# microsoft/MaskFlownet

Hardware: NVIDIA H100
Metric: image-pairs/sec (MaskFlownet-S forward, 1024x448) (higher is better)
Workload: dtype f32

## Files before the change

maskflownet_b200/csrc/api.cu:

```cuda
#include <atomic>
#include <cstdarg>
#include <cstdio>
#include <cstring>

#include "common.cuh"

namespace mfn {

static thread_local char g_err[512] = "";
static thread_local const char* g_kernel = "";
static std::atomic<unsigned long long> g_launches{0};

int fail(int code, const char* fmt, ...) {
  va_list ap;
  va_start(ap, fmt);
  vsnprintf(g_err, sizeof(g_err), fmt, ap);
  va_end(ap);
  return code;
}

void note_kernel(const char* name) { g_kernel = name; }

Tuning& tuning() {
  static Tuning t;
  return t;
}

int check_launch(const char* kernel_name) {
  const cudaError_t e = cudaGetLastError();
  if (e != cudaSuccess) return fail((int)e, "%s: launch failed: %s", kernel_name, cudaGetErrorString(e));
  g_kernel = kernel_name;
  g_launches.fetch_add(1, std::memory_order_relaxed);
  g_err[0] = '\0';
  return MFN_OK;
}

}

extern "C" int mfn_version(void) { return MFN_VERSION; }
extern "C" const char* mfn_last_error(void) { return mfn::g_err; }
extern "C" const char* mfn_last_kernel(void) { return mfn::g_kernel; }
extern "C" unsigned long long mfn_launch_count(void) { return mfn::g_launches.load(std::memory_order_relaxed); }

extern "C" int mfn_set_tuning(const char* key, int value) {
  if (!key) return mfn::fail(MFN_ERR_INVALID_ARG, "mfn_set_tuning: null key");
  if (!strcmp(key, "corr_grid_cap")) mfn::tuning().corr_grid_cap = value;
  else if (!strcmp(key, "corr_disable_ring")) mfn::tuning().corr_disable_ring = value;
  else if (!strcmp(key, "warp_lin")) mfn::tuning().warp_lin = value;
  else if (!strcmp(key, "corr_rb")) mfn::tuning().corr_rb = value;
  else if (!strcmp(key, "warp_lin_fch")) mfn::tuning().warp_lin_fch = value;
  else if (!strcmp(key, "conv_as")) mfn::tuning().conv_as = value;
  else if (!strcmp(key, "conv_splitk")) mfn::tuning().conv_splitk = value;
  else if (!strcmp(key, "conv_narrow")) mfn::tuning().conv_narrow = value;
  else if (!strcmp(key, "conv_tma_in")) mfn::tuning().conv_tma_in = value;
  else if (!strcmp(key, "corr_rb_twb")) mfn::tuning().corr_rb_twb = value;
  else if (!strcmp(key, "corr_rb_rows")) mfn::tuning().corr_rb_rows = value;
  else if (!strcmp(key, "corr_tma")) mfn::tuning().corr_tma = value;
  else if (!strcmp(key, "corr_ts_lo")) mfn::tuning().corr_ts_lo = value;
  else if (!strcmp(key, "corr_ts_hi")) mfn::tuning().corr_ts_hi = value;
  else if (!strcmp(key, "corr_dbg")) mfn::tuning().corr_dbg = value;
  else if (!strcmp(key, "conv_dbg")) mfn::tuning().conv_dbg = value;
  else if (!strcmp(key, "corr_ring_th")) mfn::tuning().corr_ring_th = value;
  else if (!strcmp(key, "conv_wgmma")) mfn::tuning().conv_wgmma = value;
  else if (!strcmp(key, "conv_grid_cap")) mfn::tuning().conv_grid_cap = value;
  else if (!strcmp(key, "conv_wgmma_min_w")) mfn::tuning().conv_wgmma_min_w = value;
  else return mfn::fail(MFN_ERR_INVALID_ARG, "mfn_set_tuning: unknown key '%s'", key);
  return MFN_OK;
}
```

maskflownet_b200/csrc/common.cuh:

```cuda
#pragma once
#include <cuda_runtime.h>
#include <stdint.h>

#include "../../include/maskflow_b200.h"
#include "device_caps.h"
#include "sampling.cuh"

namespace mfn {

int fail(int code, const char* fmt, ...);
int check_launch(const char* kernel_name);
void note_kernel(const char* name);

struct Tuning {
  int corr_grid_cap = 0;
  int corr_disable_ring = 0;
  int conv_wgmma = 1;
  int conv_grid_cap = 0;
  int conv_wgmma_min_w = 1;
  int corr_ring_th = 8;
  int corr_rb = 1;
  int warp_lin_fch = 0;
  int conv_as = 0;
  int conv_splitk = 1;
  int conv_narrow = 1;
  int conv_tma_in = 1;
  int corr_rb_twb = 0;
  int corr_rb_rows = 0;
  int corr_tma = 1;
  int warp_lin = 1;
  int corr_ts_lo = 0, corr_ts_hi = 0;
  int corr_dbg = 0;
  int conv_dbg = 0;
};
Tuning& tuning();

static inline cudaStream_t as_stream(void* s) { return reinterpret_cast<cudaStream_t>(s); }

#define MFN_REQUIRE(cond, code, ...)                   \
  do {                                                 \
    if (!(cond)) return ::mfn::fail(code, __VA_ARGS__); \
  } while (0)

static inline bool aligned(const void* p, size_t a) { return (reinterpret_cast<uintptr_t>(p) % a) == 0; }

static inline unsigned grid_for(long long total, int threads) {
  long long b = (total + threads - 1) / threads;
  const long long cap = (long long)kNumSMs * 16;
  return (unsigned)(b < cap ? (b > 0 ? b : 1) : cap);
}


struct SmemOptIn {
  int bytes[64] = {};
};
template <typename K>
static inline cudaError_t ensure_dyn_smem(K kernel, int bytes, SmemOptIn& st) {
  int dev = 0;
  if (cudaGetDevice(&dev) != cudaSuccess) dev = -1;
  if (dev >= 0 && dev < 64 && st.bytes[dev] >= bytes) return cudaSuccess;
  const cudaError_t e = cudaFuncSetAttribute(kernel, cudaFuncAttributeMaxDynamicSharedMemorySize, bytes);
  if (e == cudaSuccess && dev >= 0 && dev < 64) st.bytes[dev] = bytes;
  return e;
}

long long warp_lin_workspace_bytes(int N, int F, int H, int W);
int launch_warp_lin(const float* x, const float* flow_c, const float* mask_c, const float* weight, const void* packed_weight,
                    const float* bias, const float* tradeoff, void* workspace, float* out, float* fup, float* mup, int N,
                    int C, int H, int W, int F, int up, float fs, float ls, float slope, int border_mode, cudaStream_t st);

int launch_corr_rb(int md, const float* d1, const float* d2, float* out, int N, int C, int H, int W, long long obs,
                   float slope, cudaStream_t st);

int launch_corr_tma(int md, const float* d1, const float* d2, float* out, int N, int C, int H, int W, long long obs,
                    float slope, cudaStream_t st);

int det_launch_abs_max(const float* v, long long n, unsigned* bound, cudaStream_t st);
int det_launch_pixel_abs_sum_max(const float* g, int N, int F, long long HW, unsigned* bound, cudaStream_t st);
int det_launch_fixed_to_float(const unsigned long long* acc, float* out, long long n, const unsigned* bound, int nb,
// ... 75 lines not shown
```

maskflownet_b200/csrc/conv3x3_wgmma.cu:

```cuda
#include <cstring>
#include <type_traits>

#include "mma_tiles.cuh"
#include "split_act.cuh"

namespace mfn {
namespace um {
constexpr int MT_WIDE = 128, MT_NARROW = 64;
inline int tile_width(int OW, int stride) {
  return tuning().conv_narrow && (OW <= MT_NARROW || (stride == 2 && tuning().conv_tma_in)) ? MT_NARROW : MT_WIDE;
}
constexpr int R = 2;
constexpr int NTHREADS = 384;
constexpr int NCONS = 8;
constexpr int NPROD = 3;
constexpr int MAX_AS = 4, MAX_WS = 24;
constexpr int MAX_RS = 4;
constexpr int BATCH = 6;
constexpr int BAR_BYTES = 1024;

__host__ __device__ inline int n_slots(int stride, int dil) { return stride == 2 ? 2 * R + 1 : (dil >= R ? 3 * R : R + 2 * dil); }
__host__ __device__ inline int row_pitch(int mt, int stride, int dil) { return stride == 2 ? 2 * mt + 1 : mt + 2 * dil; }
__host__ __device__ inline int slot_of(int r, int ky, int stride, int dil) {
  return stride == 2 ? 2 * r + ky : (dil >= R ? ky * R + r : r + ky * dil);
// ... 56 lines not shown
  static_assert(S >= 32, "accumulator too small");
  asm volatile(
      "{\n\t.reg .pred p;\n\tsetp.ne.b32 p, %34, 0;\n\t"
      "wgmma.mma_async.sync.aligned.m64n64k16.f32.bf16.bf16 {%0, %1, %2, %3, %4, %5, %6, %7, %8, %9, %10, %11, %12, %13, %14, %15, %16, %17, %18, %19, %20, %21, %22, %23, %24, %25, %26, %27, %28, %29, %30, %31}, %32, %33, p, 1, 1, 0, 0;\n\t}"
      : "+f"(d[0]), "+f"(d[1]), "+f"(d[2]), "+f"(d[3]), "+f"(d[4]), "+f"(d[5]), "+f"(d[6]), "+f"(d[7]), "+f"(d[8]), "+f"(d[9]), "+f"(d[10]), "+f"(d[11]), "+f"(d[12]), "+f"(d[13]), "+f"(d[14]), "+f"(d[15]), "+f"(d[16]), "+f"(d[17]), "+f"(d[18]), "+f"(d[19]), "+f"(d[20]), "+f"(d[21]), "+f"(d[22]), "+f"(d[23]), "+f"(d[24]), "+f"(d[25]), "+f"(d[26]), "+f"(d[27]), "+f"(d[28]), "+f"(d[29]), "+f"(d[30]), "+f"(d[31])
      : "l"(a), "l"(b), "r"(scale_d));
}
template <int S>
__device__ __forceinline__ void wgmma_n80(float (&d)[S], uint64_t a, uint64_t b, uint32_t scale_d) {
  static_assert(S >= 40, "accumulator too small");
  asm volatile(
      "{\n\t.reg .pred p;\n\tsetp.ne.b32 p, %42, 0;\n\t"
      "wgmma.mma_async.sync.aligned.m64n80k16.f32.bf16.bf16 {%0, %1, %2, %3, %4, %5, %6, %7, %8, %9, %10, %11, %12, %13, %14, %15, %16, %17, %18, %19, %20, %21, %22, %23, %24, %25, %26, %27, %28, %29, %30, %31, %32, %33, %34, %35, %36, %37, %38, %39}, %40, %41, p, 1, 1, 0, 0;\n\t}"
      : "+f"(d[0]), "+f"(d[1]), "+f"(d[2]), "+f"(d[3]), "+f"(d[4]), "+f"(d[5]), "+f"(d[6]), "+f"(d[7]), "+f"(d[8]), "+f"(d[9]), "+f"(d[10]), "+f"(d[11]), "+f"(d[12]), "+f"(d[13]), "+f"(d[14]), "+f"(d[15]), "+f"(d[16]), "+f"(d[17]), "+f"(d[18]), "+f"(d[19]), "+f"(d[20]), "+f"(d[21]), "+f"(d[22]), "+f"(d[23]), "+f"(d[24]), "+f"(d[25]), "+f"(d[26]), "+f"(d[27]), "+f"(d[28]), "+f"(d[29]), "+f"(d[30]), "+f"(d[31]), "+f"(d[32]), "+f"(d[33]), "+f"(d[34]), "+f"(d[35]), "+f"(d[36]), "+f"(d[37]), "+f"(d[38]), "+f"(d[39])
      : "l"(a), "l"(b), "r"(scale_d));
}
template <int S>
__device__ __forceinline__ void wgmma_n96(float (&d)[S], uint64_t a, uint64_t b, uint32_t scale_d) {
  static_assert(S >= 48, "accumulator too small");
  asm volatile(
      "{\n\t.reg .pred p;\n\tsetp.ne.b32 p, %50, 0;\n\t"
      "wgmma.mma_async.sync.aligned.m64n96k16.f32.bf16.bf16 {%0, %1, %2, %3, %4, %5, %6, %7, %8, %9, %10, %11, %12, %13, %14, %15, %16, %17, %18, %19, %20, %21, %22, %23, %24, %25, %26, %27, %28, %29, %30, %31, %32, %33, %34, %35, %36, %37, %38, %39, %40, %41, %42, %43, %44, %45, %46, %47}, %48, %49, p, 1, 1, 0, 0;\n\t}"
      : "+f"(d[0]), "+f"(d[1]), "+f"(d[2]), "+f"(d[3]), "+f"(d[4]), "+f"(d[5]), "+f"(d[6]), "+f"(d[7]), "+f"(d[8]), "+f"(d[9]), "+f"(d[10]), "+f"(d[11]), "+f"(d[12]), "+f"(d[13]), "+f"(d[14]), "+f"(d[15]), "+f"(d[16]), "+f"(d[17]), "+f"(d[18]), "+f"(d[19]), "+f"(d[20]), "+f"(d[21]), "+f"(d[22]), "+f"(d[23]), "+f"(d[24]), "+f"(d[25]), "+f"(d[26]), "+f"(d[27]), "+f"(d[28]), "+f"(d[29]), "+f"(d[30]), "+f"(d[31]), "+f"(d[32]), "+f"(d[33]), "+f"(d[34]), "+f"(d[35]), "+f"(d[36]), "+f"(d[37]), "+f"(d[38]), "+f"(d[39]), "+f"(d[40]), "+f"(d[41]), "+f"(d[42]), "+f"(d[43]), "+f"(d[44]), "+f"(d[45]), "+f"(d[46]), "+f"(d[47])
      : "l"(a), "l"(b), "r"(scale_d));
}
template <int S>
__device__ __forceinline__ void wgmma_n112(float (&d)[S], uint64_t a, uint64_t b, uint32_t scale_d) {
  static_assert(S >= 56, "accumulator too small");
  asm volatile(
      "{\n\t.reg .pred p;\n\tsetp.ne.b32 p, %58, 0;\n\t"
      "wgmma.mma_async.sync.aligned.m64n112k16.f32.bf16.bf16 {%0, %1, %2, %3, %4, %5, %6, %7, %8, %9, %10, %11, %12, %13, %14, %15, %16, %17, %18, %19, %20, %21, %22, %23, %24, %25, %26, %27, %28, %29, %30, %31, %32, %33, %34, %35, %36, %37, %38, %39, %40, %41, %42, %43, %44, %45, %46, %47, %48, %49, %50, %51, %52, %53, %54, %55}, %56, %57, p, 1, 1, 0, 0;\n\t}"
      : "+f"(d[0]), "+f"(d[1]), "+f"(d[2]), "+f"(d[3]), "+f"(d[4]), "+f"(d[5]), "+f"(d[6]), "+f"(d[7]), "+f"(d[8]), "+f"(d[9]), "+f"(d[10]), "+f"(d[11]), "+f"(d[12]), "+f"(d[13]), "+f"(d[14]), "+f"(d[15]), "+f"(d[16]), "+f"(d[17]), "+f"(d[18]), "+f"(d[19]), "+f"(d[20]), "+f"(d[21]), "+f"(d[22]), "+f"(d[23]), "+f"(d[24]), "+f"(d[25]), "+f"(d[26]), "+f"(d[27]), "+f"(d[28]), "+f"(d[29]), "+f"(d[30]), "+f"(d[31]), "+f"(d[32]), "+f"(d[33]), "+f"(d[34]), "+f"(d[35]), "+f"(d[36]), "+f"(d[37]), "+f"(d[38]), "+f"(d[39]), "+f"(d[40]), "+f"(d[41]), "+f"(d[42]), "+f"(d[43]), "+f"(d[44]), "+f"(d[45]), "+f"(d[46]), "+f"(d[47]), "+f"(d[48]), "+f"(d[49]), "+f"(d[50]), "+f"(d[51]), "+f"(d[52]), "+f"(d[53]), "+f"(d[54]), "+f"(d[55])
      : "l"(a), "l"(b), "r"(scale_d));
}
template <int S>
__device__ __forceinline__ void wgmma_n128(float (&d)[S], uint64_t a, uint64_t b, uint32_t scale_d) {
  static_assert(S >= 64, "accumulator too small");
  asm volatile(
      "{\n\t.reg .pred p;\n\tsetp.ne.b32 p, %66, 0;\n\t"
      "wgmma.mma_async.sync.aligned.m64n128k16.f32.bf16.bf16 {%0, %1, %2, %3, %4, %5, %6, %7, %8, %9, %10, %11, %12, %13, %14, %15, %16, %17, %18, %19, %20, %21, %22, %23, %24, %25, %26, %27, %28, %29, %30, %31, %32, %33, %34, %35, %36, %37, %38, %39, %40, %41, %42, %43, %44, %45, %46, %47, %48, %49, %50, %51, %52, %53, %54, %55, %56, %57, %58, %59, %60, %61, %62, %63}, %64, %65, p, 1, 1, 0, 0;\n\t}"
      : "+f"(d[0]), "+f"(d[1]), "+f"(d[2]), "+f"(d[3]), "+f"(d[4]), "+f"(d[5]), "+f"(d[6]), "+f"(d[7]), "+f"(d[8]), "+f"(d[9]), "+f"(d[10]), "+f"(d[11]), "+f"(d[12]), "+f"(d[13]), "+f"(d[14]), "+f"(d[15]), "+f"(d[16]), "+f"(d[17]), "+f"(d[18]), "+f"(d[19]), "+f"(d[20]), "+f"(d[21]), "+f"(d[22]), "+f"(d[23]), "+f"(d[24]), "+f"(d[25]), "+f"(d[26]), "+f"(d[27]), "+f"(d[28]), "+f"(d[29]), "+f"(d[30]), "+f"(d[31]), "+f"(d[32]), "+f"(d[33]), "+f"(d[34]), "+f"(d[35]), "+f"(d[36]), "+f"(d[37]), "+f"(d[38]), "+f"(d[39]), "+f"(d[40]), "+f"(d[41]), "+f"(d[42]), "+f"(d[43]), "+f"(d[44]), "+f"(d[45]), "+f"(d[46]), "+f"(d[47]), "+f"(d[48]), "+f"(d[49]), "+f"(d[50]), "+f"(d[51]), "+f"(d[52]), "+f"(d[53]), "+f"(d[54]), "+f"(d[55]), "+f"(d[56]), "+f"(d[57]), "+f"(d[58]), "+f"(d[59]), "+f"(d[60]), "+f"(d[61]), "+f"(d[62]), "+f"(d[63])
      : "l"(a), "l"(b), "r"(scale_d));
}
template <int N, int S>
__device__ __forceinline__ void wgmma_bf16(float (&d)[S], uint64_t a, uint64_t b, uint32_t scale_d) {
  if constexpr (N == 16) wgmma_n16(d, a, b, scale_d);
  else if constexpr (N == 32) wgmma_n32(d, a, b, scale_d);
  else if constexpr (N == 48) wgmma_n48(d, a, b, scale_d);
  else if constexpr (N == 64) wgmma_n64(d, a, b, scale_d);
  else if constexpr (N == 80) wgmma_n80(d, a, b, scale_d);
  else if constexpr (N == 96) wgmma_n96(d, a, b, scale_d);
  else if constexpr (N == 112) wgmma_n112(d, a, b, scale_d);
  else wgmma_n128(d, a, b, scale_d);
}

struct SplitK {
  int k, from, n_lo, y_lo, rh;
  long long part_stride;
  float* ws;
  uint32_t magic_tp, magic_tx;
  int as_wide;
  int ns;
  int stg;
};
__device__ __forceinline__ void decode_tile(int tile, int tilesX, int tilesY, const SplitK& sk, int& tx, int& ty, int& n) {
  if (sk.magic_tp) {
    n = (int)__umulhi((uint32_t)tile, sk.magic_tp);
    const int rem = tile - n * tilesX * tilesY;
    ty = sk.magic_tx ? (int)__umulhi((uint32_t)rem, sk.magic_tx) : rem;
    tx = rem - ty * tilesX;
  } else {
    tx = tile % tilesX;
    ty = (tile / tilesX) % tilesY;
    n = tile / (tilesX * tilesY);
  }
}
struct SplitDev {
  int in, in_g0, in_Cg;
  unsigned char* out;
  int out_Cg, out_c0;
};
struct Work {
  int tile, part, cb, ce, nh;
};
__device__ __forceinline__ Work decode_work(int w, const SplitK& sk, int nChunks) {
  Work r;
  r.nh = 0;
  if (sk.ns == 2) {
    r.nh = w & 1;
    w >>= 1;
  }
  if (sk.k <= 1 || w < sk.from) {
    r.tile = w; r.part = -1; r.cb = 0; r.ce = nChunks;
  } else {
    const int u = w - sk.from, t = u / sk.k;
    r.tile = sk.from + t;
    r.part = u - t * sk.k;
    r.cb = r.part * nChunks / sk.k;
    r.ce = (r.part + 1) * nChunks / sk.k;
  }
  return r;
}

struct SmemMap {
  int a_lo, a_stage, w_tile, w_stage, w_off, bar_off, stg_off, total, AS, WS, raw_off, raw_stage, RS;
};
// ... 12 lines not shown
    const int raw_off = (2 * m.a_stage + 127) / 128 * 128;
    m.RS = rs_max;
    while (m.RS > 2 && budget - raw_off - m.RS * raw < 3 * m.w_stage) --m.RS;
    budget -= m.RS * raw + (raw_off - 2 * m.a_stage);
  }
  if (raw)
    m.AS = 2;
  else if (taps_per_stage(CoutP) > 1)
    m.AS = (4 * m.a_stage + 4 * m.w_stage <= budget) ? 4 : ((3 * m.a_stage + 3 * m.w_stage <= budget) ? 3 : 2);
  else
    m.AS = (as_wide >= 3 && 3 * m.a_stage + 8 * m.w_stage <= budget) ? 3 : 2;
  int ws = (budget - m.AS * m.a_stage) / m.w_stage;
  m.WS = ws > MAX_WS ? MAX_WS : ws;
  m.raw_off = raw ? (m.AS * m.a_stage + 127) / 128 * 128 : m.AS * m.a_stage;
  m.raw_stage = raw;
  m.w_off = m.raw_off + m.RS * raw;
  m.bar_off = m.w_off + m.WS * m.w_stage;
  m.stg_off = m.bar_off + BAR_BYTES;
  m.total = m.stg_off + stg;
  return m;
}
}

__global__ void conv3x3_pack_wgmma_kernel(const float* __restrict__ w, unsigned char* __restrict__ packed, int Cin, int Cout,
                                          int CoutP, int nChunks16) {
  const long long total = (long long)nChunks16 * 9 * CoutP * 8;
  for (long long i = (long long)blockIdx.x * blockDim.x + threadIdx.x; i < total; i += (long long)gridDim.x * blockDim.x) {
    const int j = (int)(i & 7);
    const int f = (int)((i >> 3) % CoutP);
    const int tap = (int)((i / (8LL * CoutP)) % 9);
    const int c = (int)(i / (8LL * CoutP * 9));
    const int ch = 16 * c + 2 * j;
    float a = 0.f, b = 0.f;
    if (f < Cout) {
      if (ch < Cin) a = w[((size_t)f * Cin + ch) * 9 + tap];
      if (ch + 1 < Cin) b = w[((size_t)f * Cin + ch + 1) * 9 + tap];
    }
    uint32_t hi, lo;
    split_pair(a, b, hi, lo);
    const int wt = 64 * CoutP;
    unsigned char* tile = packed + ((size_t)c * 9 + tap) * wt;
    if (um::fold_hi_lo(CoutP)) {
      const int off = (j >> 2) * (2 * CoutP * 16) + f * 16 + (j & 3) * 4;
      *reinterpret_cast<uint32_t*>(tile + off) = hi;
      *reinterpret_cast<uint32_t*>(tile + CoutP * 16 + off) = lo;
    } else {
      const int off = (j >> 2) * (CoutP * 16) + f * 16 + (j & 3) * 4;
      *reinterpret_cast<uint32_t*>(tile + off) = hi;
      *reinterpret_cast<uint32_t*>(tile + wt / 2 + off) = lo;
    }
  }
}

template <int NW, bool FOLD, int TPS, int TERMS, int MT>
__global__ void __launch_bounds__(um::NTHREADS, 1)
    conv3x3_wgmma_kernel(const float* __restrict__ x, long long x_bs, const unsigned char* __restrict__ wpack,
                         const float* __restrict__ bias_arg, float* __restrict__ out_base, long long out_bs, int Cin, int H, int W,
                         int OH, int OW, int Cout, int CoutP, int nChunks, float slope_arg, int tilesX, int tilesY, int numWork,
                         int stride, int dil, int out_mode_arg, int ext, um::SplitK sk, um::SplitDev xs,
                         const __grid_constant__ CUtensorMap tmx, int dbg) {
  using namespace um;
  static_assert(TERMS == 1 || TERMS == 3, "one or three products per multiply-add");
  static_assert(MT == MT_WIDE || MT == MT_NARROW, "128- or 64-pixel tile rows");
  constexpr bool FOLD_ACC = FOLD && TERMS == 3;
  constexpr int P = TERMS == 1 ? 1 : 2;
  constexpr int NCOL = FOLD_ACC ? NW / 2 : NW;
  constexpr int MB = MT / 64;
  const int out_mode_k = out_mode_arg & 0xff, lin_prefix_k = out_mode_arg >> 8;
  extern __shared__ __align__(128) unsigned char smem[];
  const int nslots = n_slots(stride, dil), PW = row_pitch(MT, stride, dil), E = nslots * PW;
  const SmemMap sm = smem_map(E, CoutP, sk.as_wide, sk.stg, TERMS, xs.in == 2 ? raw_stage_bytes(nslots, MT, stride) : 0,
                              raw_ring_max(stride));
  const int AS = sm.AS, WS = sm.WS, RS = sm.RS;
  const uint32_t s_base = smem_u32(smem);
  const uint32_t bar0 = s_base + sm.bar_off;
  const uint32_t a_full = bar0, a_empty = bar0 + 8 * MAX_AS, w_full = bar0 + 16 * MAX_AS, w_empty = w_full + 8 * MAX_WS;
  const uint32_t r_full = w_empty + 8 * MAX_WS, r_empty = r_full + 8 * MAX_RS;

  const int tid = threadIdx.x, lane = tid & 31;
  const int warp = __shfl_sync(0xffffffffu, tid >> 5, 0);
  const size_t plane = (size_t)H * W;

  if (tid == 0) {
    for (int i = 0; i < AS; ++i) {
      mbar_init(a_full + 8 * i, xs.in == 1 ? 1 : NPROD);
      mbar_init(a_empty + 8 * i, NCONS);
    }
    for (int i = 0; i < RS; ++i) {
      mbar_init(r_full + 8 * i, 1);
      mbar_init(r_empty + 8 * i, NPROD);
    }
    for (int i = 0; i < WS; ++i) {
      mbar_init(w_full + 8 * i, 1);
      mbar_init(w_empty + 8 * i, NCONS);
    }
    asm volatile("fence.mbarrier_init.release.cluster;" ::: "memory");
  }
  __syncthreads();

  if (warp < 8) {
    const int r = warp >> 2, wq = warp & 3;
    const uint32_t a_lbo = (uint32_t)E * 16u, b_lbo = (uint32_t)(FOLD_ACC ? 2 * CoutP : CoutP) * 16u;
    uint32_t a_off[9];
#pragma unroll
    for (int tap = 0; tap < 9; ++tap)
      a_off[tap] = (uint32_t)(slot_of(r, tap / 3, stride, dil) * PW + tap_xoff(MT, tap % 3, stride, dil));
    const uint64_t dh_a = desc_hi(a_lbo, 128u), dh_b = desc_hi(b_lbo, 128u);
    uint32_t as = 0, aph = 0, ws = 0, wph = 0;
    const uint32_t a_lo16 = (uint32_t)sm.a_lo >> 4, a_stage16 = (uint32_t)sm.a_stage >> 4, s_base16 = s_base >> 4;
    const uint32_t w_base16 = (s_base + (uint32_t)sm.w_off) >> 4, w_tile16 = (uint32_t)sm.w_tile >> 4, w_half16 = w_tile16 >> 1;
    const uint32_t w_stage16 = (uint32_t)sm.w_stage >> 4;
    int rel_w = -1, rel_a = -1;
    auto release = [&]() {
      if (lane == 0) {
        if (rel_w >= 0) mbar_arrive(w_empty + 8 * rel_w);
        if (rel_a >= 0) mbar_arrive(a_empty + 8 * rel_a);
      }
      rel_w = rel_a = -1;
    };
    float acc[MB][NW / 2];
    for (int work = blockIdx.x; work < numWork; work += gridDim.x) {
      const Work wk = decode_work(work, sk, nChunks);
      const int cb = wk.cb, ce = wk.ce;
      const uint32_t b_nh16 = (uint32_t)(wk.nh * NCOL);
#pragma unroll
      for (int mh = 0; mh < MB; ++mh) fence_acc(acc[mh]);
      if (dbg & 8) {
        for (int c = cb; c < ce; ++c) {
          mbar_wait(a_full + 8 * as, aph);
          for (int tap = 0; tap < 9; ++tap) {
            if (tap % TPS == 0) mbar_wait(w_full + 8 * ws, wph);
            release();
            if (tap % TPS == TPS - 1) {
              rel_w = (int)ws;
              if (++ws == (uint32_t)WS) { ws = 0; wph ^= 1; }
            }
            if (tap == 8) rel_a = (int)as;
          }
          if (++as == (uint32_t)AS) { as = 0; aph ^= 1; }
        }
      }
      for (int c = (dbg & 8) ? ce : cb; c < ce; ++c) {
        mbar_wait(a_full + 8 * as, aph);
        const uint32_t a_st16 = s_base16 + as * a_stage16;
#pragma unroll
        for (int tap = 0; tap < 9; ++tap) {
          if (tap % TPS == 0) mbar_wait(w_full + 8 * ws, wph);
          const uint32_t w16 = w_base16 + ws * w_stage16 + (uint32_t)(tap % TPS) * w_tile16 + b_nh16;
          const uint64_t b_hi = dh_b | (uint64_t)w16, b_lo = dh_b | (uint64_t)(w16 + w_half16);
          const uint32_t sc = (tap == 0 && c == cb) ? 0u : 1u;
          wgmma_fence();
#pragma unroll
          for (int mh = 0; mh < MB; ++mh) {
// ... 190 lines not shown
                bulk_g2s(dst + (uint32_t)(t * sm.w_tile + run), src + t * gt + 2 * run, (uint32_t)run, w_full + 8 * ws);
              } else {
                bulk_g2s(dst + (uint32_t)(t * sm.w_tile), src + t * gt, (uint32_t)sm.w_tile, w_full + 8 * ws);
              }
            }
            if (++ws == (uint32_t)WS) { ws = 0; wph ^= 1; wrapped = true; }
          }
        }
      }
    }
  } else {
    if (xs.in == 1) {
      if (warp == 9 && lane == 0) {
        uint32_t as = 0, aph = 0;
        bool wrapped = false;
        for (int work = blockIdx.x; work < numWork; work += gridDim.x) {
          const Work wk = decode_work(work, sk, nChunks);
          int tx, ty, n;
          decode_tile(wk.tile, tilesX, tilesY, sk, tx, ty, n);
          const int x0 = tx * MT - dil, y0 = ty * R;
          const int gb = n * P * xs.in_Cg + xs.in_g0;
          for (int c = wk.cb; c < wk.ce; ++c) {
            if (wrapped) mbar_wait(a_empty + 8 * as, aph ^ 1);
            const uint32_t bar = a_full + 8 * as, dst = s_base + as * (uint32_t)sm.a_stage;
            if (dbg & 16) {
              mbar_arrive(bar);
            } else {
              mbar_arrive_expect_tx(bar, (uint32_t)sm.a_stage);
              const int g = gb + 2 * c;
              if (dil < R) {
                tma_load_4d(dst, &tmx, 0, x0, y0 - dil, g, bar);
                if constexpr (P == 2) tma_load_4d(dst + (uint32_t)sm.a_lo, &tmx, 0, x0, y0 - dil, g + xs.in_Cg, bar);
              } else if constexpr (P == 1) {
#pragma unroll 1
                for (int k = 0; k < 6; ++k) {
                  const int ky = k >> 1, kc = k & 1;
                  tma_load_4d(dst + (uint32_t)((kc * E + ky * R * PW) * 16), &tmx, 0, x0, y0 + (ky - 1) * dil, g + kc, bar);
                }
              } else {
#pragma unroll 1
                for (int k = 0; k < 12; ++k) {
                  const int ky = k >> 2, kc = (k >> 1) & 1, pl = k & 1;
                  tma_load_4d(dst + (uint32_t)(pl * sm.a_lo + (kc * E + ky * R * PW) * 16), &tmx, 0, x0, y0 + (ky - 1) * dil,
                              g + kc + pl * xs.in_Cg, bar);
                }
              }
            }
            if (++as == (uint32_t)AS) { as = 0; aph ^= 1; wrapped = true; }
          }
        }
      }
      return;
    }
    if (dbg & 16) {
      uint32_t as = 0, aph = 0;
      bool wrapped = false;
      for (int work = blockIdx.x; work < numWork; work += gridDim.x) {
        const Work wk = decode_work(work, sk, nChunks);
        for (int c = wk.cb; c < wk.ce; ++c) {
          if (wrapped) mbar_wait(a_empty + 8 * as, aph ^ 1);
          __syncwarp();
          if (lane == 0) mbar_arrive(a_full + 8 * as);
          if (++as == (uint32_t)AS) { as = 0; aph ^= 1; wrapped = true; }
        }
      }
      return;
    }
    const int pw = warp - 9;
    const int G = (E + 31) / 32;
    const bool one_plane = Cin <= 8;
    const int nItems = one_plane ? G : 2 * G;
    const int nb = (nItems + NPROD * BATCH - 1) / (NPROD * BATCH);
    const uint32_t pw_magic = 0xFFFFFFFFu / (uint32_t)PW + 1u;
    if (one_plane) {
      for (int st = 0; st < AS; ++st)
        for (int e = pw * 32 + lane; e < E; e += NPROD * 32) {
          unsigned char* d = smem + st * sm.a_stage + (E + e) * 16;
          *reinterpret_cast<uint4*>(d) = make_uint4(0u, 0u, 0u, 0u);
          if constexpr (P == 2) *reinterpret_cast<uint4*>(d + sm.a_lo) = make_uint4(0u, 0u, 0u, 0u);
        }
    }
    if (xs.in == 2) {
      const bool s2 = stride == 2;
      const int RP = raw_pitch(MT, stride), CP = nslots * RP;
      const int RPC = s2 && !one_plane ? 2 : 1;
      const uint32_t raw_bytes = (uint32_t)sm.raw_stage, raw_base = s_base + (uint32_t)sm.raw_off;
      const bool issuer = warp == 9 && lane == 0;
      int i_work = blockIdx.x, i_c = 0, i_h = 0, i_ce = 0, i_x = 0, i_y = 0, i_n = 0;
      auto i_tile = [&]() {
        if (i_work >= numWork) return;
        const Work wk = decode_work(i_work, sk, nChunks);
        int tx, ty;
        decode_tile(wk.tile, tilesX, tilesY, sk, tx, ty, i_n);
        i_c = wk.cb;
        i_ce = wk.ce;
        i_x = s2 ? 2 * tx * MT - 4 : tx * MT - 4;
        i_y = s2 ? 2 * ty * R - 1 : ty * R - 1;
      };
      auto issue = [&](uint32_t slot) {
        if (i_work >= numWork) return;
        const uint32_t bar = r_full + 8 * slot;
        if (dbg & 2) {
          mbar_arrive(bar);
        } else {
          mbar_arrive_expect_tx(bar, raw_bytes);
          tma_load_4d(raw_base + slot * raw_bytes, &tmx, i_x, i_y, 16 * i_c + 8 * i_h, i_n, bar);
// ... 324 lines not shown
  const int as_wide = tuning().conv_as == 2 ? 2 : 3;
  const bool staged = (out_mode & 0xff) == 0 && ext == 0 &&
                      (xs.out != nullptr ? (out_mode >> 8) == 0 : OW % 4 == 0 && out_bs % 4 == 0 && aligned(out, 16)) &&
                      smem_map(E, CoutP, as_wide, STG_BYTES, terms).WS >= 2;
  int raw = 0;
  const bool raw_geometry = stride == 1 ? dil == 1 && MT == MT_WIDE : MT == MT_NARROW && OW > MT_NARROW;
  if (sio.in == nullptr && tuning().conv_tma_in && raw_geometry && ext == 0 && W % 4 == 0 && x_bs % 4 == 0 &&
      aligned(x, 16)) {
    raw = raw_stage_bytes(n_slots(stride, 1), MT, stride);
    if (smem_map(E, CoutP, as_wide, staged ? STG_BYTES : 0, terms, raw, raw_ring_max(stride)).WS < 3) raw = 0;
  }
  if (raw) {
    EncodeTiledFn fn = encode_tiled_fn();
    if (fn == nullptr) return fail(MFN_ERR_UNSUPPORTED, "cuTensorMapEncodeTiled is not available from this driver");
    const cuuint64_t dim[4] = {(cuuint64_t)W, (cuuint64_t)H, (cuuint64_t)Cin, (cuuint64_t)N};
    const cuuint64_t strides[3] = {(cuuint64_t)W * 4, (cuuint64_t)W * H * 4, (cuuint64_t)x_bs * 4};
    const cuuint32_t box[4] = {(cuuint32_t)raw_pitch(MT, stride), (cuuint32_t)n_slots(stride, 1),
                               (cuuint32_t)raw_channels(stride), 1};
    const cuuint32_t es[4] = {1, 1, 1, 1};
    const CUresult r = fn(&tmx, CU_TENSOR_MAP_DATA_TYPE_FLOAT32, 4, const_cast<float*>(x), dim, strides, box, es,
                          CU_TENSOR_MAP_INTERLEAVE_NONE, CU_TENSOR_MAP_SWIZZLE_NONE, CU_TENSOR_MAP_L2_PROMOTION_L2_256B,
                          CU_TENSOR_MAP_FLOAT_OOB_FILL_NONE);
    if (r != CUDA_SUCCESS) return fail(MFN_ERR_UNSUPPORTED, "cuTensorMapEncodeTiled failed (CUresult %d)", (int)r);
    xs.in = 2;
  }
  const SmemMap sm = smem_map(E, CoutP, as_wide, staged ? STG_BYTES : 0, terms, raw, raw_ring_max(stride));
  if (sm.WS < 2 || E * 16 > 0x3FFF * 16) return -1;
  if ((long long)H * W >= (1LL << 27)) return -1;
  const int tilesX = (OW + MT - 1) / MT, tilesY = (OH + R - 1) / R;
  const int ns = CoutP > 128 ? 2 : 1;
  SplitK sk = {1, 0, 0, 0, 0, 0, nullptr, 0u, 0u, 3, ns};
  if (ws != nullptr && ext == 0) {
    sk = plan_split(N, Cin, H, W, Cout, stride, dil, tuning().conv_grid_cap);
    if (sk.k > 1 && ws_bytes < sk.k * sk.part_stride * 4) sk.k = 1;
    sk.ws = ws;
  }
  const long long tiles = (long long)N * tilesX * tilesY;
  if (tiles * ns >= (1LL << 30)) return -1;
  sk.as_wide = as_wide;
  sk.stg = staged ? STG_BYTES : 0;
  if (sk.k <= 1) sk.from = (int)tiles;
  {
    const unsigned long long tp = (unsigned long long)tilesX * tilesY;
    if ((unsigned long long)tiles * tp < (1ull << 32) && tp * tilesX < (1ull << 32)) {
      sk.magic_tp = (uint32_t)(((1ull << 32) + tp - 1) / tp);
      sk.magic_tx = tilesX == 1 ? 0u : (uint32_t)(((1ull << 32) + tilesX - 1) / tilesX);
    }
    if (tp == 1) sk.magic_tp = 0;
  }
  const long long numWork = (sk.from + (tiles - sk.from) * sk.k) * ns;
  const int cap = tuning().conv_grid_cap > 0 ? tuning().conv_grid_cap : kNumSMs;
  const unsigned grid = (unsigned)(numWork < cap ? numWork : cap);
  const char* name = terms == 3 ? "conv3x3_wgmma_kernel<CoutP=256>" : "conv3x3_wgmma_kernel<CoutP=256,bf16>";
  auto launch = [&](auto mt) -> cudaError_t {
    constexpr int M = decltype(mt)::value;
    static SmemOptIn opt[8], opt1[8];
    cudaError_t e = cudaSuccess;
    if (terms == 3) {
      e = ensure_dyn_smem(conv3x3_wgmma_kernel<32, true, 9, 3, M>, sm.total, opt[0]);
      if (e == cudaSuccess) e = ensure_dyn_smem(conv3x3_wgmma_kernel<64, true, 9, 3, M>, sm.total, opt[1]);
      if (e == cudaSuccess) e = ensure_dyn_smem(conv3x3_wgmma_kernel<96, true, 3, 3, M>, sm.total, opt[2]);
      if (e == cudaSuccess) e = ensure_dyn_smem(conv3x3_wgmma_kernel<128, true, 3, 3, M>, sm.total, opt[3]);
      if (e == cudaSuccess) e = ensure_dyn_smem(conv3x3_wgmma_kernel<80, false, 1, 3, M>, sm.total, opt[4]);
      if (e == cudaSuccess) e = ensure_dyn_smem(conv3x3_wgmma_kernel<96, false, 1, 3, M>, sm.total, opt[5]);
      if (e == cudaSuccess) e = ensure_dyn_smem(conv3x3_wgmma_kernel<112, false, 1, 3, M>, sm.total, opt[6]);
      if (e == cudaSuccess) e = ensure_dyn_smem(conv3x3_wgmma_kernel<128, false, 1, 3, M>, sm.total, opt[7]);
    } else {
      e = ensure_dyn_smem(conv3x3_wgmma_kernel<16, true, 9, 1, M>, sm.total, opt1[0]);
      if (e == cudaSuccess) e = ensure_dyn_smem(conv3x3_wgmma_kernel<32, true, 9, 1, M>, sm.total, opt1[1]);
      if (e == cudaSuccess) e = ensure_dyn_smem(conv3x3_wgmma_kernel<48, true, 3, 1, M>, sm.total, opt1[2]);
      if (e == cudaSuccess) e = ensure_dyn_smem(conv3x3_wgmma_kernel<64, true, 3, 1, M>, sm.total, opt1[3]);
      if (e == cudaSuccess) e = ensure_dyn_smem(conv3x3_wgmma_kernel<80, false, 1, 1, M>, sm.total, opt1[4]);
      if (e == cudaSuccess) e = ensure_dyn_smem(conv3x3_wgmma_kernel<96, false, 1, 1, M>, sm.total, opt1[5]);
      if (e == cudaSuccess) e = ensure_dyn_smem(conv3x3_wgmma_kernel<112, false, 1, 1, M>, sm.total, opt1[6]);
      if (e == cudaSuccess) e = ensure_dyn_smem(conv3x3_wgmma_kernel<128, false, 1, 1, M>, sm.total, opt1[7]);
    }
    if (e != cudaSuccess) return e;
#define MFN_WGMMA_LAUNCH(NW_, FOLD_, TPS_, TERMS_)                                                                      \
  conv3x3_wgmma_kernel<NW_, FOLD_, TPS_, TERMS_, M><<<grid, NTHREADS, sm.total, st>>>(                                 \
      x, x_bs, wpack, bias, out, out_bs, Cin, H, W, OH, OW, Cout, CoutP, nChunks, slope, tilesX, tilesY, (int)numWork, \
      stride, dil, out_mode, ext, sk, xs, tmx, tuning().conv_dbg)
    if (terms == 3) {
      switch (CoutP) {
        case 16: MFN_WGMMA_LAUNCH(32, true, 9, 3); name = "conv3x3_wgmma_kernel<CoutP=16,fold>"; break;
        case 32: MFN_WGMMA_LAUNCH(64, true, 9, 3); name = "conv3x3_wgmma_kernel<CoutP=32,fold>"; break;
        case 48: MFN_WGMMA_LAUNCH(96, true, 3, 3); name = "conv3x3_wgmma_kernel<CoutP=48,fold>"; break;
        case 64: MFN_WGMMA_LAUNCH(128, true, 3, 3); name = "conv3x3_wgmma_kernel<CoutP=64,fold>"; break;
        case 80: MFN_WGMMA_LAUNCH(80, false, 1, 3); name = "conv3x3_wgmma_kernel<CoutP=80>"; break;
        case 96: MFN_WGMMA_LAUNCH(96, false, 1, 3); name = "conv3x3_wgmma_kernel<CoutP=96>"; break;
        case 112: MFN_WGMMA_LAUNCH(112, false, 1, 3); name = "conv3x3_wgmma_kernel<CoutP=112>"; break;
        case 128: MFN_WGMMA_LAUNCH(128, false, 1, 3); name = "conv3x3_wgmma_kernel<CoutP=128>"; break;
        default: MFN_WGMMA_LAUNCH(128, false, 1, 3);
      }
    } else {
      switch (CoutP) {
        case 16: MFN_WGMMA_LAUNCH(16, true, 9, 1); name = "conv3x3_wgmma_kernel<CoutP=16,fold,bf16>"; break;
        case 32: MFN_WGMMA_LAUNCH(32, true, 9, 1); name = "conv3x3_wgmma_kernel<CoutP=32,fold,bf16>"; break;
        case 48: MFN_WGMMA_LAUNCH(48, true, 3, 1); name = "conv3x3_wgmma_kernel<CoutP=48,fold,bf16>"; break;
        case 64: MFN_WGMMA_LAUNCH(64, true, 3, 1); name = "conv3x3_wgmma_kernel<CoutP=64,fold,bf16>"; break;
        case 80: MFN_WGMMA_LAUNCH(80, false, 1, 1); name = "conv3x3_wgmma_kernel<CoutP=80,bf16>"; break;
        case 96: MFN_WGMMA_LAUNCH(96, false, 1, 1); name = "conv3x3_wgmma_kernel<CoutP=96,bf16>"; break;
        case 112: MFN_WGMMA_LAUNCH(112, false, 1, 1); name = "conv3x3_wgmma_kernel<CoutP=112,bf16>"; break;
        case 128: MFN_WGMMA_LAUNCH(128, false, 1, 1); name = "conv3x3_wgmma_kernel<CoutP=128,bf16>"; break;
        default: MFN_WGMMA_LAUNCH(128, false, 1, 1);
      }
    }
#undef MFN_WGMMA_LAUNCH
    return cudaSuccess;
  };
  const cudaError_t e = MT == MT_NARROW ? launch(std::integral_constant<int, MT_NARROW>{})
                                        : launch(std::integral_constant<int, MT_WIDE>{});
  if (e != cudaSuccess) return fail((int)e, "cudaFuncSetAttribute(conv3x3_wgmma_kernel): %s", cudaGetErrorString(e));
  const int rc = check_launch(name);
  if (rc != 0 || sk.k <= 1) return rc;
  const long long total = sk.part_stride;
  long long blocks = (total + 255) / 256;
  if (blocks > 4 * kNumSMs) blocks = 4 * kNumSMs;
  if (terms == 3) {
    conv3x3_wgmma_reduce_kernel<3><<<(unsigned)blocks, 256, 0, st>>>(sk, xs, N - sk.n_lo, bias, out, out_bs, Cout, OH, OW, slope, out_mode);
    return check_launch("conv3x3_wgmma_reduce_kernel");
  }
  conv3x3_wgmma_reduce_kernel<1><<<(unsigned)blocks, 256, 0, st>>>(sk, xs, N - sk.n_lo, bias, out, out_bs, Cout, OH, OW, slope, out_mode);
  return check_launch("conv3x3_wgmma_reduce_kernel<bf16>");
}

}
```

maskflownet_b200/csrc/ptx.cuh:

```cuda
#pragma once
#include <cuda.h>
#include <cstdint>

#include "bf16_split.cuh"

namespace mfn {

__device__ __forceinline__ uint32_t smem_u32(const void* p) { return (uint32_t)__cvta_generic_to_shared(p); }

__device__ __forceinline__ void ldsm_x4(uint32_t addr, uint32_t (&r)[4]) {
  asm volatile("ldmatrix.sync.aligned.m8n8.x4.shared.b16 {%0,%1,%2,%3}, [%4];"
               : "=r"(r[0]), "=r"(r[1]), "=r"(r[2]), "=r"(r[3])
               : "r"(addr)
               : "memory");
}

__device__ __forceinline__ void mma_bf16(float (&d)[4], const uint32_t (&a)[4], uint32_t b0, uint32_t b1) {
  asm volatile(
      "mma.sync.aligned.m16n8k16.row.col.f32.bf16.bf16.f32 {%0,%1,%2,%3}, {%4,%5,%6,%7}, {%8,%9}, {%0,%1,%2,%3};"
      : "+f"(d[0]), "+f"(d[1]), "+f"(d[2]), "+f"(d[3])
      : "r"(a[0]), "r"(a[1]), "r"(a[2]), "r"(a[3]), "r"(b0), "r"(b1));
}

__host__ __device__ __forceinline__ int swz(int p, int c) { return p * 64 + ((c ^ ((p >> 1) & 3)) << 4); }

__device__ __forceinline__ void cp_async16(uint32_t dst, const void* src) {
  asm volatile("cp.async.cg.shared.global [%0], [%1], 16;" ::"r"(dst), "l"(src) : "memory");
}
__device__ __forceinline__ void cp_async_commit() { asm volatile("cp.async.commit_group;" ::: "memory"); }
template <int N>
__device__ __forceinline__ void cp_async_wait() { asm volatile("cp.async.wait_group %0;" ::"n"(N) : "memory"); }

__device__ __forceinline__ void mbar_init(uint32_t bar, uint32_t count) {
  asm volatile("mbarrier.init.shared::cta.b64 [%0], %1;" ::"r"(bar), "r"(count) : "memory");
}
__device__ __forceinline__ void mbar_arrive(uint32_t bar) {
  asm volatile("{\n\t.reg .b64 st;\n\tmbarrier.arrive.shared::cta.b64 st, [%0];\n\t}" ::"r"(bar) : "memory");
}
__device__ __forceinline__ void mbar_arrive_n(uint32_t bar, uint32_t n) {
  asm volatile("{\n\t.reg .b64 st;\n\tmbarrier.arrive.shared::cta.b64 st, [%0], %1;\n\t}" ::"r"(bar), "r"(n) : "memory");
}
__device__ __forceinline__ void mbar_arrive_expect_tx(uint32_t bar, uint32_t bytes) {
  asm volatile("{\n\t.reg .b64 st;\n\tmbarrier.arrive.expect_tx.shared::cta.b64 st, [%0], %1;\n\t}" ::"r"(bar), "r"(bytes)
               : "memory");
}
__device__ __forceinline__ void mbar_wait(uint32_t bar, uint32_t parity) {
  uint32_t done = 0, spins = 0;
  while (!done) {
    asm volatile(
        "{\n\t.reg .pred p;\n\tmbarrier.try_wait.parity.shared::cta.b64 p, [%1], %2;\n\tselp.u32 %0, 1, 0, p;\n\t}"
        : "=r"(done)
        : "r"(bar), "r"(parity)
        : "memory");
    if (!done && ++spins > (1u << 28)) __trap();
  }
}

__device__ __forceinline__ void bulk_g2s(uint32_t dst, const void* src, uint32_t bytes, uint32_t bar) {
  asm volatile("cp.async.bulk.shared::cluster.global.mbarrier::complete_tx::bytes [%0], [%1], %2, [%3];" ::"r"(dst),
               "l"(src), "r"(bytes), "r"(bar)
               : "memory");
}
__device__ __forceinline__ void bulk_s2g(void* dst, uint32_t src, uint32_t bytes) {
  asm volatile("cp.async.bulk.global.shared::cta.bulk_group [%0], [%1], %2;" ::"l"(dst), "r"(src), "r"(bytes) : "memory");
}
__device__ __forceinline__ void bulk_commit() { asm volatile("cp.async.bulk.commit_group;" ::: "memory"); }
__device__ __forceinline__ void bulk_wait_read() { asm volatile("cp.async.bulk.wait_group.read 0;" ::: "memory"); }
__device__ __forceinline__ void bulk_wait_all() { asm volatile("cp.async.bulk.wait_group 0;" ::: "memory"); }

__device__ __forceinline__ void tma_load_4d(uint32_t dst, const CUtensorMap* tm, int c0, int c1, int c2, int c3,
                                            uint32_t bar) {
  asm volatile(
      "cp.async.bulk.tensor.4d.shared::cluster.global.tile.mbarrier::complete_tx::bytes [%0], [%1, {%2, %3, %4, %5}], [%6];" ::
          "r"(dst),
      "l"(tm), "r"(c0), "r"(c1), "r"(c2), "r"(c3), "r"(bar)
      : "memory");
}
__device__ __forceinline__ void tma_store_4d(const CUtensorMap* tm, uint32_t src, int c0, int c1, int c2, int c3) {
  asm volatile("cp.async.bulk.tensor.4d.global.shared::cta.tile.bulk_group [%0, {%2, %3, %4, %5}], [%1];" ::"l"(tm),
               "r"(src), "r"(c0), "r"(c1), "r"(c2), "r"(c3)
               : "memory");
}

__device__ __forceinline__ void named_bar_sync(int id, int nthreads) {
  asm volatile("bar.sync %0, %1;" ::"r"(id), "r"(nthreads) : "memory");
}

}
```

Measured before the change: 829.0.

## Add weights-in-registers wgmma consumer path for CoutP=128 wide conv3x3

Adds a specialized conv3x3 consumer path that loads weight fragments from shared memory into registers via ldmatrix and issues register-sourced wgmma (A from registers, activations via a shared-memory descriptor). Weight fragments for the next tap are double-buffered while the current tap's MMAs run. Register budgets are rebalanced with setmaxnreg between producer and consumer warps. The aim is to cut shared-memory descriptor traffic for weights and the per-tap pipeline overhead on CoutP=128 layers, at the cost of register pressure (R×64 accumulators plus fragments) and a new, more complex code path. It is on by default when the eligibility conditions hold.

```diff
diff --git a/maskflownet_b200/csrc/api.cu b/maskflownet_b200/csrc/api.cu
--- a/maskflownet_b200/csrc/api.cu
+++ b/maskflownet_b200/csrc/api.cu
@@ -53,6 +53,7 @@
   else if (!strcmp(key, "conv_splitk")) mfn::tuning().conv_splitk = value;
   else if (!strcmp(key, "conv_narrow")) mfn::tuning().conv_narrow = value;
   else if (!strcmp(key, "conv_tma_in")) mfn::tuning().conv_tma_in = value;
+  else if (!strcmp(key, "conv_wreg")) mfn::tuning().conv_wreg = value;
   else if (!strcmp(key, "corr_rb_twb")) mfn::tuning().corr_rb_twb = value;
   else if (!strcmp(key, "corr_rb_rows")) mfn::tuning().corr_rb_rows = value;
   else if (!strcmp(key, "corr_tma")) mfn::tuning().corr_tma = value;
diff --git a/maskflownet_b200/csrc/common.cuh b/maskflownet_b200/csrc/common.cuh
--- a/maskflownet_b200/csrc/common.cuh
+++ b/maskflownet_b200/csrc/common.cuh
@@ -25,6 +25,7 @@
   int conv_splitk = 1;
   int conv_narrow = 1;
   int conv_tma_in = 1;
+  int conv_wreg = 1;
   int corr_rb_twb = 0;
   int corr_rb_rows = 0;
   int corr_tma = 1;
diff --git a/maskflownet_b200/csrc/conv3x3_wgmma.cu b/maskflownet_b200/csrc/conv3x3_wgmma.cu
--- a/maskflownet_b200/csrc/conv3x3_wgmma.cu
+++ b/maskflownet_b200/csrc/conv3x3_wgmma.cu
@@ -132,6 +132,16 @@
   else if constexpr (N == 96) wgmma_n96(d, a, b, scale_d);
   else if constexpr (N == 112) wgmma_n112(d, a, b, scale_d);
   else wgmma_n128(d, a, b, scale_d);
+}
+
+template <int S>
+__device__ __forceinline__ void wgmma_rs_n128(float (&d)[S], const uint32_t (&a)[4], uint64_t b, uint32_t scale_d) {
+  static_assert(S >= 64, "accumulator too small");
+  asm volatile(
+      "{\n\t.reg .pred p;\n\tsetp.ne.b32 p, %69, 0;\n\t"
+      "wgmma.mma_async.sync.aligned.m64n128k16.f32.bf16.bf16 {%0, %1, %2, %3, %4, %5, %6, %7, %8, %9, %10, %11, %12, %13, %14, %15, %16, %17, %18, %19, %20, %21, %22, %23, %24, %25, %26, %27, %28, %29, %30, %31, %32, %33, %34, %35, %36, %37, %38, %39, %40, %41, %42, %43, %44, %45, %46, %47, %48, %49, %50, %51, %52, %53, %54, %55, %56, %57, %58, %59, %60, %61, %62, %63}, {%64, %65, %66, %67}, %68, p, 1, 1, 0;\n\t}"
+      : "+f"(d[0]), "+f"(d[1]), "+f"(d[2]), "+f"(d[3]), "+f"(d[4]), "+f"(d[5]), "+f"(d[6]), "+f"(d[7]), "+f"(d[8]), "+f"(d[9]), "+f"(d[10]), "+f"(d[11]), "+f"(d[12]), "+f"(d[13]), "+f"(d[14]), "+f"(d[15]), "+f"(d[16]), "+f"(d[17]), "+f"(d[18]), "+f"(d[19]), "+f"(d[20]), "+f"(d[21]), "+f"(d[22]), "+f"(d[23]), "+f"(d[24]), "+f"(d[25]), "+f"(d[26]), "+f"(d[27]), "+f"(d[28]), "+f"(d[29]), "+f"(d[30]), "+f"(d[31]), "+f"(d[32]), "+f"(d[33]), "+f"(d[34]), "+f"(d[35]), "+f"(d[36]), "+f"(d[37]), "+f"(d[38]), "+f"(d[39]), "+f"(d[40]), "+f"(d[41]), "+f"(d[42]), "+f"(d[43]), "+f"(d[44]), "+f"(d[45]), "+f"(d[46]), "+f"(d[47]), "+f"(d[48]), "+f"(d[49]), "+f"(d[50]), "+f"(d[51]), "+f"(d[52]), "+f"(d[53]), "+f"(d[54]), "+f"(d[55]), "+f"(d[56]), "+f"(d[57]), "+f"(d[58]), "+f"(d[59]), "+f"(d[60]), "+f"(d[61]), "+f"(d[62]), "+f"(d[63])
+      : "r"(a[0]), "r"(a[1]), "r"(a[2]), "r"(a[3]), "l"(b), "r"(scale_d));
 }
 
 struct SplitK {
@@ -250,7 +260,7 @@
   }
 }
 
-template <int NW, bool FOLD, int TPS, int TERMS, int MT>
+template <int NW, bool FOLD, int TPS, int TERMS, int MT, bool WREG = false>
 __global__ void __launch_bounds__(um::NTHREADS, 1)
     conv3x3_wgmma_kernel(const float* __restrict__ x, long long x_bs, const unsigned char* __restrict__ wpack,
                          const float* __restrict__ bias_arg, float* __restrict__ out_base, long long out_bs, int Cin, int H, int W,
@@ -296,7 +306,171 @@
   }
   __syncthreads();
 
-  if (warp < 8) {
+  if constexpr (WREG) {
+    static_assert(NW == 128 && !FOLD && TPS == 1 && MT == MT_WIDE, "the weights-from-registers consumer: CoutP = 128, wide tiles");
+    if (warp >= 8) {
+      setmaxnreg_dec<40>();
+    } else {
+      setmaxnreg_inc<232>();
+      const int g = warp >> 2, wq = warp & 3;
+      uint32_t x_off[9];
+#pragma unroll
+      for (int tap = 0; tap < 9; ++tap)
+        x_off[tap] = (uint32_t)(slot_of(0, tap / 3, 1, dil) * PW + tap_xoff(MT, tap % 3, 1, dil));
+      const uint64_t dh_x = desc_hi((uint32_t)E * 16u, 128u);
+      const uint32_t a_lo16 = (uint32_t)sm.a_lo >> 4, a_stage16 = (uint32_t)sm.a_stage >> 4, s_base16 = s_base >> 4;
+      const uint32_t w_lane = s_base + (uint32_t)sm.w_off + (uint32_t)(((lane >> 4) * CoutP + 64 * g + 16 * wq + (lane & 15)) * 16);
+      uint32_t as = 0, aph = 0, ws = 0, wph = 0;
+      int rel_a = -1;
+      auto release_a = [&]() {
+        if (rel_a >= 0 && lane == 0) mbar_arrive(a_empty + 8 * rel_a);
+        rel_a = -1;
+      };
+      auto next_w = [&]() {
+        if (++ws == (uint32_t)WS) { ws = 0; wph ^= 1; }
+      };
+      auto load_w = [&](uint32_t (&f)[P][4]) {
+        mbar_wait<true>(w_full + 8 * ws, wph);
+        const uint32_t a = w_lane + ws * (uint32_t)sm.w_stage;
+        ldsm_x4(a, f[0]);
+        if constexpr (P == 2) ldsm_x4(a + (uint32_t)(sm.w_tile >> 1), f[1]);
+        __syncwarp();
+        if (lane == 0) mbar_arrive(w_empty + 8 * ws);
+        next_w();
+      };
+      uint32_t wf[2][P][4];
+      float acc[R][64];
+      for (int work = blockIdx.x; work < numWork; work += gridDim.x) {
+#pragma unroll
+        for (int rr = 0; rr < R; ++rr) fence_acc(acc[rr]);
+        auto chunk = [&](auto par, const bool first, const bool last) {
+          constexpr int PAR = decltype(par)::value;
+          mbar_wait<true>(a_full + 8 * as, aph);
+          const uint32_t x_st16 = s_base16 + as * a_stage16;
+#pragma unroll
+          for (int tap = 0; tap < 9; ++tap) {
+            const uint32_t (&cur)[P][4] = wf[(tap + PAR) & 1];
+            const uint32_t sc = (tap == 0 && first) ? 0u : 1u;
+            wgmma_fence();
+#pragma unroll
+            for (int rr = 0; rr < R; ++rr) {
+              const uint32_t x16 = x_st16 + x_off[tap] + (uint32_t)(rr * PW);
+              const uint64_t x_hi = dh_x | (uint64_t)x16, x_lo = dh_x | (uint64_t)(x16 + a_lo16);
+              if constexpr (TERMS == 1) {
+                wgmma_rs_n128(acc[rr], cur[0], x_hi, sc);
+              } else {
+                wgmma_rs_n128(acc[rr], cur[P - 1], x_hi, sc);
+                wgmma_rs_n128(acc[rr], cur[0], x_lo, 1u);
+                wgmma_rs_n128(acc[rr], cur[0], x_hi, 1u);
+              }
+            }
+            wgmma_commit();
+            wgmma_wait<1>();
+            release_a();
+            if (tap < 8 || !last) load_w(wf[(tap + PAR + 1) & 1]);
+            if (tap == 8) rel_a = (int)as;
+          }
+          if (++as == (uint32_t)AS) { as = 0; aph ^= 1; }
+        };
+        if (dbg & 8) {
+          for (int c = 0; c < nChunks; ++c) {
+            mbar_wait<true>(a_full + 8 * as, aph);
+            for (int tap = 0; tap < 9; ++tap) {
+              mbar_wait<true>(w_full + 8 * ws, wph);
+              release_a();
+              if (lane == 0) mbar_arrive(w_empty + 8 * ws);
+              next_w();
+              if (tap == 8) rel_a = (int)as;
+            }
+            if (++as == (uint32_t)AS) { as = 0; aph ^= 1; }
+          }
+        } else {
+          load_w(wf[0]);
+          for (int c = 0; c < nChunks; ++c) {
+            if (c & 1) chunk(std::integral_constant<int, 1>{}, false, c == nChunks - 1);
+            else chunk(std::integral_constant<int, 0>{}, c == 0, c == nChunks - 1);
+          }
+        }
+        wgmma_wait<0>();
+#pragma unroll
+        for (int rr = 0; rr < R; ++rr) fence_acc(acc[rr]);
+        release_a();
+
+        if (dbg & 4) continue;
+        int tx, ty, n;
+        decode_tile(work, tilesX, tilesY, sk, tx, ty, n);
+        const size_t oplane0 = (size_t)OH * OW;
+        const int t = wq * 32 + lane, q = lane >> 2, pp = lane & 3;
+        const int x0 = tx * MT;
+        const uint32_t seg = (uint32_t)((OW - x0 < MT ? OW - x0 : MT) * 4);
+        float* const stg = reinterpret_cast<float*>(smem + sm.stg_off) + g * STG_CH * SPITCH;
+        float bv[2];
+#pragma unroll
+        for (int h = 0; h < 2; ++h) {
+          const int f = 64 * g + 16 * wq + q + 8 * h;
+          bv[h] = (bias_arg != nullptr && f < Cout) ? __ldg(bias_arg + f) : 0.f;
+        }
+#pragma unroll
+        for (int rr = 0; rr < R; ++rr) {
+          const int y = ty * R + rr;
+          if (y >= OH) continue;
+#pragma unroll
+          for (int h = 0; h < 2; ++h) {
+            if (xs.out != nullptr) {
+              unsigned char* const sst = reinterpret_cast<unsigned char*>(stg);
+              if (t < 4 * P) bulk_wait_read();
+              named_bar_sync(1 + g, 128);
+              const bool odd = q & 1;
+              unsigned char* const row = sst + (wq * P * MT + 2 * pp + (odd ? 1 : 0)) * 16 + (q >> 1) * 4;
+#pragma unroll
+              for (int j = 0; j < 16; ++j) {
+                const float v0 = leaky(acc[rr][4 * j + 2 * h] + bv[h], slope_arg);
+                const float v1 = leaky(acc[rr][4 * j + 2 * h + 1] + bv[h], slope_arg);
+                const float o = __shfl_xor_sync(0xffffffffu, odd ? v0 : v1, 4);
+                const float ve = odd ? o : v0, vo = odd ? v1 : o;
+                unsigned char* const e = row + 8 * j * 16;
+                if constexpr (TERMS == 1) {
+                  *reinterpret_cast<uint32_t*>(e) = bf16_pair(ve, vo);
+                } else {
+                  uint32_t hi, lo;
+                  split_pair(ve, vo, hi, lo);
+                  *reinterpret_cast<uint32_t*>(e) = hi;
+                  *reinterpret_cast<uint32_t*>(e + MT * 16) = lo;
+                }
+              }
+              asm volatile("fence.proxy.async.shared::cta;" ::: "memory");
+              named_bar_sync(1 + g, 128);
+              const int f = 64 * g + 16 * (t >> (P - 1)) + 8 * h;
+              if (t < 4 * P && f < Cout) {
+                const long long dst = sa::entry<P>(n, t & (P - 1), (xs.out_c0 + f) >> 3, (long long)y * OW + x0, xs.out_Cg,
+                                                   oplane0);
+                bulk_s2g(xs.out + dst, smem_u32(sst + t * MT * 16), seg * 4);
+                bulk_commit();
+              }
+            } else {
+              if (t < STG_CH) bulk_wait_read();
+              named_bar_sync(1 + g, 128);
+              float* const row = stg + (8 * wq + (((q & 3) << 1) | (q >> 2))) * SPITCH + 2 * pp;
+#pragma unroll
+              for (int j = 0; j < 16; ++j)
+                *reinterpret_cast<float2*>(row + 8 * j) = make_float2(leaky(acc[rr][4 * j + 2 * h] + bv[h], slope_arg),
+                                                                      leaky(acc[rr][4 * j + 2 * h + 1] + bv[h], slope_arg));
+              asm volatile("fence.proxy.async.shared::cta;" ::: "memory");
+              named_bar_sync(1 + g, 128);
+              const int f = 64 * g + 16 * (t >> 3) + (((t & 7) >> 1) | ((t & 1) << 2)) + 8 * h;
+              if (t < STG_CH && f < Cout) {
+                bulk_s2g(out_base + (size_t)n * out_bs + (size_t)f * oplane0 + (size_t)y * OW + x0, smem_u32(stg + t * SPITCH), seg);
+                bulk_commit();
+              }
+            }
+          }
+        }
+      }
+      bulk_wait_all();
+      return;
+    }
+  }
+  if (!WREG && warp < 8) {
     const int r = warp >> 2, wq = warp & 3;
     const uint32_t a_lbo = (uint32_t)E * 16u, b_lbo = (uint32_t)(FOLD_ACC ? 2 * CoutP : CoutP) * 16u;
     uint32_t a_off[9];
@@ -593,6 +767,7 @@
       }
       return;
     }
+    if constexpr (WREG) return;
     if (dbg & 16) {
       uint32_t as = 0, aph = 0;
       bool wrapped = false;
@@ -1023,10 +1198,33 @@
   const int cap = tuning().conv_grid_cap > 0 ? tuning().conv_grid_cap : kNumSMs;
   const unsigned grid = (unsigned)(numWork < cap ? numWork : cap);
   const char* name = terms == 3 ? "conv3x3_wgmma_kernel<CoutP=256>" : "conv3x3_wgmma_kernel<CoutP=256,bf16>";
+  const bool wreg = tuning().conv_wreg && CoutP == 128 && MT == MT_WIDE && xs.in == 1 && staged && sk.k <= 1 && (out_mode >> 8) == 0;
   auto launch = [&](auto mt) -> cudaError_t {
     constexpr int M = decltype(mt)::value;
     static SmemOptIn opt[8], opt1[8];
     cudaError_t e = cudaSuccess;
+#define MFN_WGMMA_LAUNCH_W(NW_, FOLD_, TPS_, TERMS_, WREG_)                                                             \
+  conv3x3_wgmma_kernel<NW_, FOLD_, TPS_, TERMS_, M, WREG_><<<grid, NTHREADS, sm.total, st>>>(                          \
+      x, x_bs, wpack, bias, out, out_bs, Cin, H, W, OH, OW, Cout, CoutP, nChunks, slope, tilesX, tilesY, (int)numWork, \
+      stride, dil, out_mode, ext, sk, xs, tmx, tuning().conv_dbg)
+#define MFN_WGMMA_LAUNCH(NW_, FOLD_, TPS_, TERMS_) MFN_WGMMA_LAUNCH_W(NW_, FOLD_, TPS_, TERMS_, false)
+    if constexpr (M == MT_WIDE) {
+      if (wreg) {
+        static SmemOptIn optw[2];
+        if (terms == 3) {
+          e = ensure_dyn_smem(conv3x3_wgmma_kernel<128, false, 1, 3, M, true>, sm.total, optw[0]);
+          if (e != cudaSuccess) return e;
+          MFN_WGMMA_LAUNCH_W(128, false, 1, 3, true);
+          name = "conv3x3_wgmma_kernel<CoutP=128,wreg>";
+        } else {
+          e = ensure_dyn_smem(conv3x3_wgmma_kernel<128, false, 1, 1, M, true>, sm.total, optw[1]);
+          if (e != cudaSuccess) return e;
+          MFN_WGMMA_LAUNCH_W(128, false, 1, 1, true);
+          name = "conv3x3_wgmma_kernel<CoutP=128,wreg,bf16>";
+        }
+        return cudaSuccess;
+      }
+    }
     if (terms == 3) {
       e = ensure_dyn_smem(conv3x3_wgmma_kernel<32, true, 9, 3, M>, sm.total, opt[0]);
       if (e == cudaSuccess) e = ensure_dyn_smem(conv3x3_wgmma_kernel<64, true, 9, 3, M>, sm.total, opt[1]);
@@ -1047,10 +1245,6 @@
       if (e == cudaSuccess) e = ensure_dyn_smem(conv3x3_wgmma_kernel<128, false, 1, 1, M>, sm.total, opt1[7]);
     }
     if (e != cudaSuccess) return e;
-#define MFN_WGMMA_LAUNCH(NW_, FOLD_, TPS_, TERMS_)                                                                      \
-  conv3x3_wgmma_kernel<NW_, FOLD_, TPS_, TERMS_, M><<<grid, NTHREADS, sm.total, st>>>(                                 \
-      x, x_bs, wpack, bias, out, out_bs, Cin, H, W, OH, OW, Cout, CoutP, nChunks, slope, tilesX, tilesY, (int)numWork, \
-      stride, dil, out_mode, ext, sk, xs, tmx, tuning().conv_dbg)
     if (terms == 3) {
       switch (CoutP) {
         case 16: MFN_WGMMA_LAUNCH(32, true, 9, 3); name = "conv3x3_wgmma_kernel<CoutP=16,fold>"; break;
@@ -1077,6 +1271,7 @@
       }
     }
 #undef MFN_WGMMA_LAUNCH
+#undef MFN_WGMMA_LAUNCH_W
     return cudaSuccess;
   };
   const cudaError_t e = MT == MT_NARROW ? launch(std::integral_constant<int, MT_NARROW>{})
diff --git a/maskflownet_b200/csrc/ptx.cuh b/maskflownet_b200/csrc/ptx.cuh
--- a/maskflownet_b200/csrc/ptx.cuh
+++ b/maskflownet_b200/csrc/ptx.cuh
@@ -44,6 +44,8 @@
   asm volatile("{\n\t.reg .b64 st;\n\tmbarrier.arrive.expect_tx.shared::cta.b64 st, [%0], %1;\n\t}" ::"r"(bar), "r"(bytes)
                : "memory");
 }
+static __device__ __noinline__ void mbar_timeout() { __trap(); }
+template <bool CALL = false>
 __device__ __forceinline__ void mbar_wait(uint32_t bar, uint32_t parity) {
   uint32_t done = 0, spins = 0;
   while (!done) {
@@ -52,7 +54,10 @@
         : "=r"(done)
         : "r"(bar), "r"(parity)
         : "memory");
-    if (!done && ++spins > (1u << 28)) __trap();
+    if (!done && ++spins > (1u << 28)) {
+      if constexpr (CALL) mbar_timeout();
+      else __trap();
+    }
   }
 }
 
@@ -86,4 +91,9 @@
   asm volatile("bar.sync %0, %1;" ::"r"(id), "r"(nthreads) : "memory");
 }
 
+template <int N>
+__device__ __forceinline__ void setmaxnreg_inc() { asm volatile("setmaxnreg.inc.sync.aligned.u32 %0;" ::"n"(N)); }
+template <int N>
+__device__ __forceinline__ void setmaxnreg_dec() { asm volatile("setmaxnreg.dec.sync.aligned.u32 %0;" ::"n"(N)); }
+
 }
```

Result: no change. 830.5 (median of 6 runs) (+0.2%).
